# zhangyi-3/UCDIR

Measured on AMD Instinct MI355X. Metric: restored images/sec at 50-step p_sample_loop, 256x256 SID, higher is better.
Workload: dtype bf16

## Files before the change

### ucdir_amd/csrc/engine.hip

```cpp
#include <hip/hip_runtime.h>

#include <algorithm>
#include <cmath>
#include <cstdio>
#include <cstring>
#include <map>
#include <mutex>
#include <set>
#include <array>
#include <atomic>
#include <memory>
#include <string>
#include <vector>

#include "../../include/ucdir_hip.h"
#include "cgemm.hip.h"
#include "conv_halo.hip.h"
#include "akgm_halo.hip.h"
#include "akgm_pre.hip.h"
#include "akgm_ws.hip.h"
#include "akgm_ws32.hip.h"
#include "akgm_ws64.hip.h"
#include "conv_ws.hip.h"
#include "conv_sk.hip.h"
// ... 274 lines not shown
    sd.print([&](int, int n) { fprintf(stderr, "CGEMM TIMING mode=%d TM=%d nk=%d n=%d:", p.cols_mode, TM, p.nk, n); });
}

static int ilog2(int v) { int s = 0; while ((1 << s) < v) ++s; return s; }

static void zero_gemm(GemmP& p) { std::memset(&p, 0, sizeof(p)); p.alpha = 1.f; p.groups_per_wg = 1; }

static Act make_act(DevPool& pool, int B, int H, int W, int C, bool with_stats = true) {
    Act a; a.B = B; a.H = H; a.W = W; a.C = C;
    a.p = (bf16_t*)pool.alloc((size_t)a.elems() * sizeof(bf16_t), true);
    if (with_stats) {
        a.stats = pool.alloc_stats(B);
    }
    return a;
}

static void choose_tile(int H, int W, int& th, int& tw) {
    static std::map<std::pair<int, int>, std::pair<int, int>> memo;
    static std::mutex mu;
    std::lock_guard<std::mutex> lk(mu);
    auto it = memo.find({H, W});
    if (it != memo.end()) { th = it->second.first; tw = it->second.second; return; }
    double best = -1; th = 16; tw = 16;
    for (int a = 1; a <= 64; ++a)
        for (int b = 4; b <= 256; ++b) {
            if (a * b > 256 || (a + 2) * (b + 2) > HC_HALO_PX) continue;
            const double tiles = (double)((H + a - 1) / a) * ((W + b - 1) / b);
            const double util = (double)H * W / (tiles * 256.0) - 1e-4 * (a + 2) * (b + 2) / 324.0;
            if (util > best) { best = util; th = a; tw = b; }
        }
    memo[{H, W}] = {th, tw};
}

static std::atomic<int> g_last_ksplit{0};
template <int TM, bool DUAL = false>
static void launch_halo(GemmP p, hipStream_t st) {
    const int ks = p.ksplit > 1 ? p.ksplit : 1;
    g_last_ksplit = ks;
    const int nblk = p.nbatch * p.tiles_x * p.tiles_y * p.rowtiles * (p.up_phase ? 4 : 1) * ks + p.alt_blocks;
    ProfEntry e = gemm_entry((TM == 128 ? KEY_HALO128 : KEY_HALO64) + (p.up_phase ? KEY_HALO_UP : 0) + (DUAL ? KEY_HALO_DUAL : 0), p, EPI_STD, p.cg);
    if (p.alt_blocks) add_res_rider(e, p);
    StampDump sd(st, STAMPS_256); p.dbg = sd.dbg();
    bracket(e, st, [&] {
        hipLaunchKernelGGL((conv3x3_halo_kernel<TM, DUAL>), dim3(nblk), dim3(HC_THREADS), hc_lds_bytes<TM>(), st, p);
        if (ks == 1) return;
        const long long items = (long long)p.H * p.W * (p.up_phase ? 4 : 1) * (p.nfeat / 8);
        int gx = (int)((items + 255) / 256); if (gx > 1024) gx = 1024;
        hipLaunchKernelGGL(conv_splitk_finish_kernel, dim3(gx, p.nbatch), dim3(256), 0, st, p, TM);
    });
    sd.print([](int, int n) { fprintf(stderr, "TIMING n=%d:", n); });
}

static std::atomic<int> g_persist_grid{0};
static int num_cus() {
    if (g_persist_grid > 0) return g_persist_grid;
    static std::map<int, int> memo;
    static std::mutex mu;
    std::lock_guard<std::mutex> lk(mu);
    int dev = 0;
    HIPC(hipGetDevice(&dev));
    auto it = memo.find(dev);
    if (it != memo.end()) return it->second;
    int n = 0;
    HIPC(hipDeviceGetAttribute(&n, hipDeviceAttributeMultiprocessorCount, dev));
    if (n <= 0) n = 256;
    memo[dev] = n;
    return n;
}

static thread_local float* t_splitk = nullptr;
static float* splitk_scratch() {
    if (t_splitk) return t_splitk;
    std::lock_guard<std::mutex> lk(g_static_mu);
    int dev = 0;
    HIPC(hipGetDevice(&dev));
    auto it = g_splitk_buf.find(dev);
    if (it != g_splitk_buf.end()) return it->second;
    float* sk = nullptr;
    HIPC(hipMalloc((void**)&sk, SCRATCH_BYTES));
    g_splitk_buf[dev] = sk;
    return sk;
}
static std::atomic<int> g_splitk{-1};
static bool splitk_on() {
    return g_splitk < 0 ? env().splitk : g_splitk != 0;
}
static int choose_ksplit(int wgs, int nchunks, int steps_per_chunk, double out_elems) {
    if (!splitk_on() || wgs > env().splitk_wgs || wgs <= 0) return 1;
    const double unsplit = (double)nchunks * steps_per_chunk * (wgs > 256 ? 1.3 : 1.0);
    int best = 1;
    double best_cost = 0.85 * unsplit;
    for (int ks = 2; ks <= 16 && wgs * ks <= SPLITK_MAX_WGS && nchunks / ks >= 2; ++ks) {
        const double steps = (double)((nchunks + ks - 1) / ks) * steps_per_chunk * (wgs * ks > 256 ? 1.3 : 1.0);
        const double cost = steps + 5.0 + out_elems * 4.0 * ks / 1.5e6;
        if (cost < best_cost) { best_cost = cost; best = ks; }
    }
    return best;
}

static int choose_usplit(int nblk) {
    if (!splitk_on() || nblk <= 0) return 1;
    int best_us = 1;
    double best = 1e30;
    for (int us = 1; us <= 4; us *= 2) {
        const double cost = (double)((nblk * us + SPLITK_MAX_WGS - 1) / SPLITK_MAX_WGS) * (1.0 / us + 0.10);
        if (cost < best - 1e-9) { best = cost; best_us = us; }
// ... 827 lines not shown
    for (size_t li = 0; li < c->layers.size(); ++li) {
        const LayerDesc& d = c->layers[li];
        LayerRT& r = c->rt[li];
        for (; si < slots.size() && slots[si].layer == (int)li; ++si) {
            const ActSlot& s = slots[si];
            Act a; a.B = B; a.H = s.H; a.W = s.W; a.C = s.C;
            if (s.id == (int)bufs.size()) bufs.push_back((bf16_t*)c->apool.alloc((size_t)a.elems() * sizeof(bf16_t), true));
            a.p = bufs.at(s.id);
            if (s.which != ACT_RES) a.stats = c->apool.alloc_stats(B);
            (s.which == ACT_OUT ? r.out : s.which == ACT_H1 ? r.h1 : s.which == ACT_RES ? r.res : r.bo) = a;
        }
        if (d.kind == "stem") {
            fl += 2.0 * 9 * d.cin * d.cout * c->Hc * c->Wc;
        } else if (d.kind == "down") {
            const int h = level_dim(c->Hc, d.level + 1), w = level_dim(c->Wc, d.level + 1);
            fl += 2.0 * 9 * d.cin * d.cout * h * w;
        } else if (d.kind == "up") {
            const int h = level_dim(c->Hc, d.level - 1), w = level_dim(c->Wc, d.level - 1);
            fl += 2.0 * 9 * d.cin * d.cout * h * w;
        } else {
            const int h = level_dim(c->Hc, d.level), w = level_dim(c->Wc, d.level);
            r.G = (float*)c->apool.alloc((size_t)B * h * w * 8 * sizeof(float));
            const double hw = (double)h * w;
            fl += 2.0 * 9 * d.cin * d.cout * hw + 2.0 * 9 * d.cout * d.cout * hw;
            if (d.cin != d.cout) fl += 2.0 * d.cin * d.cout * hw;
            fl += 2.0 * hw * (3 * 16 + 72 * 8);
            if (d.attn) {
                if (h * w > maxN) maxN = h * w;
                attC = d.cout;
                fl += 2.0 * d.cout * 3 * d.cout * hw + 2.0 * d.cout * d.cout * hw + 4.0 * hw * hw * d.cout;
            }
        }
    }
    fl += 2.0 * 9 * c->cfg.inner_channel * c->cfg.channel_mults[0] * c->cfg.out_channel * c->Hc * c->Wc;
    c->flops = fl * B;
    c->fin_act = Act();
    if (!c->fin_w || env().no_fused_final) c->fin_act = make_act(c->apool, B, c->Hc, c->Wc, c->cfg.inner_channel * c->cfg.channel_mults[0], false);
    if (maxN > 0) alloc_attn(c->apool, c->attn, B, maxN, attC, c->cfg.attn_fp16 != 0);
    c->attw = (float*)c->apool.alloc((size_t)c->nblocks * B * 8 * sizeof(float));
    {
        int maxC = 0;
        for (const auto& d : c->layers) if (d.kind == "block" && d.cout > maxC) maxC = d.cout;
        c->tcbuf = (float*)c->apool.alloc((size_t)B * (9 * 8 * maxC + 2) * sizeof(float), false);
    }
    c->guide_ready = false;
}

static void forward(ucdir_ctx* c, const float* cond, const float* xt, const float* level, float* eps, hipStream_t st) {
    struct ScratchScope { ScratchScope(float* p) { t_splitk = p; } ~ScratchScope() { t_splitk = nullptr; } } scratch_scope(c->splitk);
    c->apool.zero_stats(st);
    require(c->finalized, "weights not finalized");
    require(c->guide_ready, "ucdir_prepare_guide must be called before ucdir_unet_forward");
    const int B = c->B, inner = c->cfg.inner_channel;
    {
        const size_t sm = (size_t)(6 * inner + c->nblocks * 8) * sizeof(float);
        hipLaunchKernelGGL(time_mlp_kernel, dim3(B), dim3(256), sm, st, level, inner, c->mlp_w1, c->mlp_b1, c->mlp_w2,
                           c->mlp_b2, c->tw, c->nblocks, c->attw, B);
        HIPC(hipGetLastError());
    }
    std::vector<const Act*> skips;
    const Act* cur = nullptr;
    for (size_t li = 0; li < c->layers.size(); ++li) {
        const LayerDesc& d = c->layers[li];
        const LayerW& w = c->lw[li];
        LayerRT& r = c->rt[li];
        if (d.kind == "stem") {
            const int tx = (c->Wc + 15) / 16, ty = (c->Hc + 15) / 16;
            const int units = tx * ty * (d.cout / 64) * B;
            hipLaunchKernelGGL((stem_mfma_kernel<6, 0>), dim3(units < 4 * num_cus() ? units : 4 * num_cus()), dim3(256), 0, st, cond, xt, c->H, c->W,
                               c->Hc, c->Wc, d.cout, tx, w.stem_w, r.out.p, r.out.stats, tx * ty, d.cout / 64, B);
            HIPC(hipGetLastError());
        } else if (d.kind == "down") {
            run_conv(w.conv, COLS_DOWN, {*cur, nullptr, r.out, 0, nullptr, true}, st);
        } else if (d.kind == "up") {
            run_conv(w.conv, COLS_UP, {*cur, nullptr, r.out, 0, nullptr, true}, st);
        } else {
            const Act* x0 = cur; const Act* x1 = nullptr;
            if (d.skip_c) { x1 = skips.back(); skips.pop_back(); require(x1->C == d.skip_c, "skip channel mismatch"); }
            const bool res_done = run_conv(w.conv, COLS_S1, {*x0, x1, r.h1, 1, nullptr, true, w.has_res ? &r.res : nullptr, w.has_res ? &w.resconv : nullptr}, st);
            const Act* res = x0;
            if (w.has_res) { if (!res_done) run_conv(w.resconv, COLS_S1, {*x0, x1, r.res, 0, nullptr, false}, st); res = &r.res; }
            Act& bo = d.attn ? r.bo : r.out;
            run_akgm(w.sp, r.h1, r.G, c->attw + (size_t)w.block_index * B * 8, *res, bo, c->tcbuf, st);
            if (d.attn) run_attention(w.qkv, w.outp, bo, r.out, c->attn, st);
        }
        cur = &r.out;
        if (d.push_skip) skips.push_back(cur);
    }
    {
        const int C = cur->C, co = c->cfg.out_channel;
        if (!env().no_fused_final && c->fin_w) {
            const int tiles = ((c->Wc + 15) / 16) * ((c->Hc + 15) / 16) * B;
            const dim3 grid(tiles < 3 * num_cus() ? tiles : 3 * num_cus());
            const size_t lds = (size_t)324 * 80 + (size_t)9 * (C / 32) * 1024 + (size_t)8 * C + (size_t)8 * B;
            require(lds <= 160 * 1024, "final conv: channel count too large for the fused kernel");
            hipLaunchKernelGGL(final_conv_kernel, grid, dim3(256), lds, st, cur->p, c->Hc, c->Wc, C, cur->stats,
                               1.0 / ((double)C * c->Hc * c->Wc), c->fin_gamma, c->fin_beta, c->fin_w, c->fin_b, co, eps, c->H, c->W, B);
            HIPC(hipGetLastError());
        } else {
            hipLaunchKernelGGL(gn_silu_kernel, dim3(2048, 1, B), dim3(256), 0, st, cur->p, c->fin_act.p, c->Hc, c->Wc, C,
                               cur->stats, 1.0 / ((double)C * c->Hc * c->Wc), c->fin_gamma, c->fin_beta);
            HIPC(hipGetLastError());
            Act dummy; dummy.B = B; dummy.H = c->Hc; dummy.W = c->Wc; dummy.C = c->fin_conv.cout;
            run_conv(c->fin_conv, COLS_S1, {c->fin_act, nullptr, dummy, 0, nullptr, false, nullptr, nullptr, eps, c->H, c->W}, st);
        }
    }
}

static void forward_graph(ucdir_ctx* c, const float* cond, const float* xt, const float* level, float* eps, hipStream_t st) {
    for (auto& f : c->graphs)
        if (f.cond == cond && f.xt == xt && f.lvl == level && f.eps == eps) { c->miss_streak = 0; HIPC(hipGraphLaunch(f.ex, st)); return; }
    const bool same_as_last = c->last_miss[0] == cond && c->last_miss[1] == xt && c->last_miss[2] == level && c->last_miss[3] == eps;
    c->last_miss[0] = cond; c->last_miss[1] = xt; c->last_miss[2] = level; c->last_miss[3] = eps;
    if (c->miss_streak >= 2 && !same_as_last) { ++c->miss_streak; forward(c, cond, xt, level, eps, st); return; }
    ++c->miss_streak;
    if (c->graphs.size() >= 8) { const int ms = c->miss_streak; c->drop_graphs(); c->miss_streak = ms; }
    if (!c->cap_stream) HIPC(hipStreamCreateWithFlags(&c->cap_stream, hipStreamNonBlocking));
    HIPC(hipStreamSynchronize(st));
    ucdir_ctx::FwdGraph f{cond, xt, level, eps, nullptr, nullptr};
    HIPC(hipStreamBeginCapture(c->cap_stream, hipStreamCaptureModeThreadLocal));
    try { forward(c, cond, xt, level, eps, c->cap_stream); }
    catch (...) { hipGraph_t g = nullptr; (void)hipStreamEndCapture(c->cap_stream, &g); if (g) (void)hipGraphDestroy(g); throw; }
    HIPC(hipStreamEndCapture(c->cap_stream, &f.g));
    if (hipGraphInstantiate(&f.ex, f.g, nullptr, nullptr, 0) != hipSuccess) {
        (void)hipGraphDestroy(f.g);
        throw std::runtime_error("hipGraphInstantiate failed for a captured forward");
    }
    c->graphs.push_back(f);
    HIPC(hipGraphLaunch(f.ex, st));
}

extern "C" {

int32_t ucdir_abi_version(void) { return UCDIR_ABI_VERSION; }
const char* ucdir_last_error(void) { return g_err.c_str(); }

int32_t ucdir_create(const ucdir_config* cfg, ucdir_ctx** out) {
    API_BEGIN
    require(cfg && out, "null argument");
    require(cfg->n_mults >= 1 && cfg->n_mults <= UCDIR_MAX_MULTS, "bad n_mults");
    require(cfg->inner_channel % 64 == 0, "inner_channel must be a multiple of 64");
    int ndev = 0;
    hipError_t e = hipGetDeviceCount(&ndev);
    require(e == hipSuccess && ndev > 0, "no HIP device available (libucdir_hip has no CPU fallback)");
    require(cfg->device >= 0 && cfg->device < ndev, "bad device ordinal");
    DevGuard dg(cfg->device);
    ensure_kernel_attrs();
    std::unique_ptr<ucdir_ctx> c(new ucdir_ctx());
    c->cfg = *cfg;
    c->layers = build_layers(*cfg);
    for (const auto& d : c->layers)
// ... 95 lines not shown
int32_t ucdir_set_graph(ucdir_ctx* ctx, int32_t on) {
    API_BEGIN
    require(ctx, "null ctx");
    DevGuard dg(ctx->cfg.device);
    ctx->use_graph = on != 0;
    if (!on) ctx->drop_graphs();
    API_END
}

int32_t ucdir_debug_read(ucdir_ctx* ctx, const char* layer, const char* what, float* dst, int64_t dst_elems, void* stream) {
    API_BEGIN
    require(ctx && layer && what && dst, "null argument");
    DevGuard dg(ctx->cfg.device);
    require(!ctx->acts_reused, "ucdir_debug_read: activation buffers of this (large) shape are recycled by lifetime; set "
                               "UCDIR_KEEP_ACTS=1 before planning to keep every layer's tensor");
    const bool padded = !strncmp(what, "padded:", 7);
    if (padded) what += 7;
    for (size_t li = 0; li < ctx->layers.size(); ++li) {
        if (ctx->layers[li].name != layer) continue;
        const LayerRT& r = ctx->rt[li];
        require(!padded || !strcmp(what, "out") || !strcmp(what, "h1") || !strcmp(what, "res") || !strcmp(what, "bo"),
                "debug_read: padded: takes out, h1, res or bo");
        if (!strcmp(what, "attw")) {
            require(ctx->layers[li].kind == "block" && ctx->attw != nullptr, "attw: not a residual block");
            require(dst_elems == (int64_t)ctx->B * 8, "debug_read: attw has B * 8 elements");
            HIPC(hipMemcpyAsync(dst, ctx->attw + (size_t)ctx->lw[li].block_index * ctx->B * 8, sizeof(float) * ctx->B * 8,
                                hipMemcpyDeviceToDevice, (hipStream_t)stream));
            return 0;
        }
        const Act* a = &r.out;
        if (!strcmp(what, "h1")) a = &r.h1;
        else if (!strcmp(what, "res")) a = &r.res;
        else if (!strcmp(what, "bo")) a = &r.bo;
        require(a->p != nullptr, "no such activation");
        const int64_t n = padded ? (int64_t)a->elems() : (int64_t)a->B * a->C * a->H * a->W;
        require(n == dst_elems, "debug_read: dst has " + std::to_string(dst_elems) + " elements, activation has " + std::to_string(n));
        if (padded) hipLaunchKernelGGL(act_to_nchw_padded_kernel, dim3(2048), dim3(256), 0, (hipStream_t)stream, a->p, dst, a->B, a->C, a->H, a->W);
        else hipLaunchKernelGGL(act_to_nchw_kernel, dim3(2048), dim3(256), 0, (hipStream_t)stream, a->p, dst, a->B, a->C, a->H, a->W);
        HIPC(hipGetLastError());
        return 0;
    }
    throw std::runtime_error(std::string("unknown layer ") + layer);
    API_END
}

int32_t ucdir_debug_flag(const char* name, int32_t value) {
    API_BEGIN
    require(name != nullptr, "null argument");
    if (!strcmp(name, "flash")) g_flash = value;
    else if (!strcmp(name, "splitk")) g_splitk = value;
    else if (!strcmp(name, "skmix")) g_skmix = value;
    else if (!strcmp(name, "convsk")) g_convsk = value;
    else if (!strcmp(name, "persist_grid")) g_persist_grid = value;
    else if (!strcmp(name, "reuse_acts")) g_reuse_acts = value < 0 ? -1 : value != 0;
    else throw std::runtime_error(std::string("unknown debug flag ") + name);
    API_END
}

int32_t ucdir_debug_launch_plan(const char* what, int32_t wgs, int32_t nchunks, int32_t steps_per_chunk, double out_elems) {
    if (!what) return -1;
    try {
        if (!strcmp(what, "ksplit")) return choose_ksplit(wgs, nchunks, steps_per_chunk, out_elems);
        if (!strcmp(what, "usplit")) return choose_usplit(wgs);
        if (!strcmp(what, "last_ksplit")) return g_last_ksplit;
        if (!strcmp(what, "tile")) {
            if (wgs < 1 || nchunks < 1) return -1;
            int th = 0, tw = 0;
            choose_tile(wgs, nchunks, th, tw);
            return th * 1000 + tw;
        }
        if (!strcmp(what, "sk_strips")) {
            if (wgs < 1) return -1;
            int ns = 0, Ws = 0, Wpe = 0, nhp = 0;
            bool ok;
            if (nchunks == 14) ok = conv_sk_strips<1, 4>(wgs, ns, Ws, Wpe, nhp);
            else if (nchunks == 28) ok = conv_sk_strips<2, 8>(wgs, ns, Ws, Wpe, nhp);
            else if (nchunks == 18) ok = conv_sk_strips<1, 8>(wgs, ns, Ws, Wpe, nhp);
            else return -1;
            return ok ? ns * 1000 + nhp : 0;
        }
    } catch (...) {}
    return -1;
}

int32_t ucdir_debug_act_plan(const ucdir_config* cfg, int32_t B, int32_t H, int32_t W, int32_t pad_mode, int32_t reuse, int32_t cap,
                             int32_t* rows) {
    try {
        require(cfg && (rows || cap <= 0), "null argument");
        require(cfg->n_mults >= 1 && cfg->n_mults <= UCDIR_MAX_MULTS, "bad n_mults");
        int Hc, Wc;
        plan_compute_size(*cfg, B, H, W, pad_mode, Hc, Wc);
        const std::vector<ActSlot> plan = act_plan(build_layers(*cfg), Hc, Wc, reuse_acts_mode(reuse < 0 ? -1 : reuse != 0, Hc, Wc));
        for (size_t i = 0; i < plan.size() && (int64_t)i < cap; ++i) {
            const ActSlot& s = plan[i];
            const int32_t r[6] = {s.layer, s.which, s.H, s.W, s.C, s.id};
            for (int k = 0; k < 6; ++k) rows[i * 6 + k] = r[k];
        }
        return (int32_t)plan.size();
    }
    catch (const std::exception& e) { fail(e.what()); }
    catch (...) { fail("unknown error"); }
    return -1;
}

int32_t ucdir_profile_enable(int32_t on) {
    API_BEGIN
// ... 233 lines not shown
    {
        int cinp, coutp;
        auto wp = pad_conv_weight(H_("conv10_1.weight"), 3, {32}, 1, cinp, coutp);
        std::vector<float> w3((size_t)3 * cinp); for (int o = 0; o < 3; ++o) for (int ci = 0; ci < cinp; ++ci) w3[(size_t)o * cinp + ci] = wp[(size_t)o * cinp + ci];
        c->conv["conv10_1"] = upload_conv(c->wpool, w3.data(), H_("conv10_1.bias").data(), nullptr, nullptr, 3, cinp, 1);
    }
    const int ups[4][3] = {{6, 512, 256}, {7, 256, 128}, {8, 128, 64}, {9, 64, 32}};
    for (auto& u : ups) {
        const std::string n = "upv" + std::to_string(u[0]);
        const int cin = u[1], cout = u[2], coutp = pad64(cout);
        const auto& w = H_(n + ".weight"); const auto& b = H_(n + ".bias");
        require(w.size() == (size_t)cin * cout * 4, "predictor: " + n + " size");
        std::vector<float> t((size_t)4 * coutp * cin, 0.f), bb((size_t)4 * coutp, 0.f);
        for (int q = 0; q < 4; ++q) for (int o = 0; o < cout; ++o) {
            bb[(size_t)q * coutp + o] = b[o];
            for (int ci = 0; ci < cin; ++ci) t[((size_t)q * coutp + o) * cin + ci] = w[((size_t)ci * cout + o) * 4 + q];
        }
        c->conv[n] = upload_conv(c->wpool, t.data(), bb.data(), nullptr, nullptr, 4 * coutp, cin, 1);
    }
    c->host.clear();
    c->finalized = true;
}

static void predictor_plan(ucdir_predictor* c, int B, int H, int W) {
    require(B >= 1, "predictor: B must be >= 1");
    require(H >= 33 && W >= 33, "predictor: H, W must be >= 33 (reflect pad)");
    c->apool.release(); c->act.clear();
    c->B = B; c->H = H; c->W = W; c->Hc = (H / 32 + 1) * 32; c->Wc = (W / 32 + 1) * 32;
    const int ch[5] = {64, 64, 128, 256, 512};
    for (int l = 0; l < 5; ++l) {
        const int h = c->Hc >> l, w = c->Wc >> l;
        const std::string L = std::to_string(l + 1);
        c->act["a" + L] = make_act(c->apool, B, h, w, ch[l], false);
        c->act["c" + L] = make_act(c->apool, B, h, w, ch[l], false);
        if (l < 4) c->act["p" + L] = make_act(c->apool, B, h / 2, w / 2, ch[l], false);
    }
    for (int l = 3; l >= 0; --l) {
        const int h = c->Hc >> l, w = c->Wc >> l;
        const std::string L = std::to_string(9 - l);
        c->act["u" + L] = make_act(c->apool, B, h, w, ch[l], false);
        c->act["a" + L] = make_act(c->apool, B, h, w, ch[l], false);
        c->act["c" + L] = make_act(c->apool, B, h, w, ch[l], false);
    }
}

static void predictor_forward(ucdir_predictor* c, const float* x, float* y, hipStream_t st) {
    const int B = c->B;
    auto A = [&](const std::string& n) -> Act& { return c->act.at(n); };
    auto CV = [&](const std::string& n) -> const ConvW& { return c->conv.at(n); };
    {
        const int tx = (c->Wc + 15) / 16, ty = (c->Hc + 15) / 16;
        const int units = tx * ty * B;
        hipLaunchKernelGGL((stem_mfma_kernel<3, 2>), dim3(units < 4 * num_cus() ? units : 4 * num_cus()), dim3(256), 0, st, x, x, c->H, c->W, c->Hc, c->Wc, 64, tx,
                           c->in_w, A("a1").p, (stat_t*)nullptr, tx * ty, 1, B);
        HIPC(hipGetLastError());
    }
    run_conv(CV("conv1_2"), COLS_S1, {A("a1"), nullptr, A("c1"), 2, nullptr, false}, st);
    for (int l = 1; l <= 4; ++l) {
        const std::string L = std::to_string(l), N = std::to_string(l + 1);
        Act& src = A("c" + L); Act& dst = A("p" + L);
        hipLaunchKernelGGL(maxpool2_kernel, dim3(2048), dim3(256), 0, st, src.p, dst.p, B, src.H, src.W, src.C);
        HIPC(hipGetLastError());
        run_conv(CV("conv" + N + "_1"), COLS_S1, {dst, nullptr, A("a" + N), 2, nullptr, false}, st);
        run_conv(CV("conv" + N + "_2"), COLS_S1, {A("a" + N), nullptr, A("c" + N), 2, nullptr, false}, st);
    }
    const Act* cur = &A("c5");
    for (int l = 6; l <= 9; ++l) {
        const std::string L = std::to_string(l);
        Act& up = A("u" + L);
        const ConvW& w = CV("upv" + L);
        {
            GemmP p; zero_gemm(p);
            p.A = w.A; p.a_ld = w.Kpad; p.a_rows = w.rows_pad;
            p.B0 = cur->p; p.b0_bstride = cur->bstride(); p.ld0 = cur->C; p.c0 = cur->C;
            p.cols_mode = COLS_S1; p.H = cur->H; p.W = cur->W; p.Wp = cur->W + 2; p.Hi = cur->H; p.Wi = cur->W; p.Wpi = p.Wp;
            p.p0 = p.Wp + 1; p.pn = (cur->H - 1) * p.Wp + cur->W;
            p.ntaps = 1; p.cg = cur->C; p.cpt = cur->C / 8; p.nk = w.Kpad / CG_BK;
            p.tiles = (p.pn + CG_TP - 1) / CG_TP; p.rowtiles = w.rows_pad / w.TM; p.nbatch = B;
            p.bias = w.bias; p.nfeat = w.cout; p.shuffle_c = up.C;
            p.out = up.p; p.out_bstride = up.bstride(); p.out_ld = up.C;
            launch_cgemm(p, w.TM, EPI_STD, st);
        }
        const Act& skip = A("c" + std::to_string(10 - l));
        run_conv(CV("conv" + L + "_1"), COLS_S1, {up, &skip, A("a" + L), 2, nullptr, false}, st);
        run_conv(CV("conv" + L + "_2"), COLS_S1, {A("a" + L), nullptr, A("c" + L), 2, nullptr, false}, st);
        cur = &A("c" + L);
    }
    {
        const ConvW& w = CV("conv10_1");
        GemmP p; zero_gemm(p);
        p.A = w.A; p.a_ld = w.Kpad; p.a_rows = w.rows_pad;
        p.B0 = cur->p; p.b0_bstride = cur->bstride(); p.ld0 = cur->C; p.c0 = cur->C;
        p.cols_mode = COLS_S1; p.H = cur->H; p.W = cur->W; p.Wp = cur->W + 2; p.Hi = cur->H; p.Wi = cur->W; p.Wpi = p.Wp;
        p.p0 = p.Wp + 1; p.pn = (cur->H - 1) * p.Wp + cur->W;
        p.ntaps = 1; p.cg = cur->C; p.cpt = cur->C / 8; p.nk = w.Kpad / CG_BK;
        p.tiles = (p.pn + CG_TP - 1) / CG_TP; p.rowtiles = w.rows_pad / w.TM; p.nbatch = B;
        p.bias = w.bias; p.nfeat = 3; p.out = y; p.out_nchw = 1; p.crop_h = c->H; p.crop_w = c->W;
        launch_cgemm(p, w.TM, EPI_STD, st);
    }
}

extern "C" {

int32_t ucdir_predictor_create(int32_t device, ucdir_predictor** out) {
    API_BEGIN
    require(out, "null argument");
    int ndev = 0;
// ... 80 lines not shown
```

### ucdir_amd/csrc/misc.hip.h

```cpp
#pragma once
#include "common.h"

__global__ void act_stats_kernel(const bf16_t* __restrict__ x, int H, int W, int C, stat_t* __restrict__ stats) {
    const int b = blockIdx.x;
    const int Wp = W + 2;
    const long long bs = (long long)(H + 2) * Wp * C;
    const int c8 = C / 8;
    double s1 = 0, s2 = 0;
    for (long long i = threadIdx.x; i < (long long)H * W * c8; i += blockDim.x) {
        int c = (int)(i % c8);
        long long pix = i / c8;
        int y = (int)(pix / W), xx = (int)(pix % W);
        const uint4 v = *reinterpret_cast<const uint4*>(x + b * bs + ((long long)(y + 1) * Wp + xx + 1) * C + c * 8);
        const bf16_t* h = reinterpret_cast<const bf16_t*>(&v);
#pragma unroll
        for (int k = 0; k < 8; ++k) { float f = bf2f(h[k]); s1 += f; s2 += (double)f * f; }
    }
    __shared__ double sh[2][256];
    sh[0][threadIdx.x] = s1; sh[1][threadIdx.x] = s2;
    __syncthreads();
    for (int o = 128; o > 0; o >>= 1) {
        if ((int)threadIdx.x < o) { sh[0][threadIdx.x] += sh[0][threadIdx.x + o]; sh[1][threadIdx.x] += sh[1][threadIdx.x + o]; }
        __syncthreads();
    }
    if (threadIdx.x == 0) stat_store(stats, b, sh[0][0], sh[1][0]);
}

__global__ void nchw_to_act_kernel(const float* __restrict__ src, bf16_t* __restrict__ dst, int B, int C, int H, int W) {
    long long n = (long long)B * H * W * C;
    for (long long i = blockIdx.x * (long long)blockDim.x + threadIdx.x; i < n; i += (long long)gridDim.x * blockDim.x) {
        int c = (int)(i % C); long long t = i / C;
        int x = (int)(t % W); t /= W;
        int y = (int)(t % H); int b = (int)(t / H);
        float v = src[(((long long)b * C + c) * H + y) * W + x];
        dst[(((long long)b * (H + 2) + y + 1) * (W + 2) + x + 1) * C + c] = f2bf(v);
    }
}
__global__ void act_to_nchw_kernel(const bf16_t* __restrict__ src, float* __restrict__ dst, int B, int C, int H, int W) {
    long long n = (long long)B * H * W * C;
    for (long long i = blockIdx.x * (long long)blockDim.x + threadIdx.x; i < n; i += (long long)gridDim.x * blockDim.x) {
        int x = (int)(i % W); long long t = i / W;
        int y = (int)(t % H); t /= H;
        int c = (int)(t % C); int b = (int)(t / C);
        dst[i] = bf2f(src[(((long long)b * (H + 2) + y + 1) * (W + 2) + x + 1) * C + c]);
    }
}
__global__ void act_to_nchw_padded_kernel(const bf16_t* __restrict__ src, float* __restrict__ dst, int B, int C, int H, int W) {
    const int Hp = H + 2, Wp = W + 2;
    long long n = (long long)B * Hp * Wp * C;
    for (long long i = blockIdx.x * (long long)blockDim.x + threadIdx.x; i < n; i += (long long)gridDim.x * blockDim.x) {
        int x = (int)(i % Wp); long long t = i / Wp;
        int y = (int)(t % Hp); t /= Hp;
        int c = (int)(t % C); int b = (int)(t / C);
        dst[i] = bf2f(src[(((long long)b * Hp + y) * Wp + x) * C + c]);
    }
}
__global__ void nchw8_to_compact_kernel(const float* __restrict__ src, float* __restrict__ dst, int B, int H, int W) {
    long long n = (long long)B * H * W * 8;
    for (long long i = blockIdx.x * (long long)blockDim.x + threadIdx.x; i < n; i += (long long)gridDim.x * blockDim.x) {
        int s = (int)(i % 8); long long t = i / 8;
        long long pix = t % ((long long)H * W); int b = (int)(t / ((long long)H * W));
        dst[i] = src[((long long)b * 8 + s) * H * W + pix];
    }
}

__device__ __forceinline__ int reflect_idx(int i, int n) { return i < n ? i : 2 * (n - 1) - i; }

template <int CIN, int ACT>
__global__ __launch_bounds__(256, 4) void stem_mfma_kernel(const float* __restrict__ cond, const float* __restrict__ xt,
                                                           int H, int W, int Hc, int Wc, int C0, int tiles_x,
                                                           const bf16_t* __restrict__ wfrag,
                                                           bf16_t* __restrict__ out, stat_t* __restrict__ stats_out,
                                                           int tiles, int ncb, int nb) {
    __shared__ uint4 halo[324];
    __shared__ uint4 wl[2 * 5 * 64];
    __shared__ float red[8];
    __shared__ __attribute__((aligned(16))) unsigned char otile[4 * 32 * 144];
    const int tid = threadIdx.x, lane = tid & 63, wv = tid >> 6, hh = lane >> 5;
    const int total = tiles * ncb * nb;
    auto gather = [&](int u, float (&v)[2][8]) {
        const int tile = u % tiles, b = u / (tiles * ncb);
        const int y0 = (tile / tiles_x) * 16, x0 = (tile % tiles_x) * 16;
#pragma unroll
        for (int uu = 0; uu < 2; ++uu) {
            const int hp = tid + uu * 256;
#pragma unroll
            for (int k = 0; k < 8; ++k) v[uu][k] = 0.f;
            if (hp < 324) {
                const int hr = hp / 18, hc = hp - hr * 18;
                const int yy = y0 + hr - 1, xx = x0 + hc - 1;
                if (yy >= 0 && yy < Hc && xx >= 0 && xx < Wc) {
                    const int ys = reflect_idx(yy, H), xs = reflect_idx(xx, W);
#pragma unroll
                    for (int ci = 0; ci < CIN; ++ci) {
                        const float* src = ci < 3 ? cond : xt;
                        v[uu][ci] = src[(((long long)b * 3 + (ci % 3)) * H + ys) * W + xs];
                    }
                }
            }
        }
    };
    float v[2][8];
    if ((int)blockIdx.x < total) gather(blockIdx.x, v);
    int cb_cur = -1;
#pragma unroll 1
    for (int u = blockIdx.x; u < total; u += gridDim.x) {
        const int tile = u % tiles, cb = (u / tiles) % ncb, b = u / (tiles * ncb);
        const int y0 = (tile / tiles_x) * 16, x0 = (tile % tiles_x) * 16;
        __syncthreads();
#pragma unroll
        for (int uu = 0; uu < 2; ++uu)
            if (tid + uu * 256 < 324) halo[tid + uu * 256] = pack8_bf16(v[uu]);
        if (cb != cb_cur) {
            for (int i = tid; i < 2 * 5 * 64; i += 256)
                wl[i] = *reinterpret_cast<const uint4*>(wfrag + ((long long)cb * 2 * 5 * 64 + i) * 8);
            cb_cur = cb;
        }
        if (u + (int)gridDim.x < total) gather(u + gridDim.x, v);
        __syncthreads();
        int hp0[2];
#pragma unroll
        for (int tp = 0; tp < 2; ++tp) {
            const int slot = tp * 32 + (lane & 31);
            hp0[tp] = (wv * 4 + (slot >> 4)) * 18 + (slot & 15);
        }
        f32x16_t acc[2][2];
#pragma unroll
        for (int tm = 0; tm < 2; ++tm)
#pragma unroll
            for (int tp = 0; tp < 2; ++tp)
#pragma unroll
                for (int e = 0; e < 16; ++e) acc[tm][tp][e] = 0.f;
#pragma unroll 1
        for (int j = 0; j < 5; ++j) {
            const int t0 = 2 * j, t1 = (2 * j + 1 > 8) ? 8 : 2 * j + 1;
            const int sh = hh ? (t1 / 3) * 18 + (t1 % 3) : (t0 / 3) * 18 + (t0 % 3);
            bf16x8_t af[2], bfr[2];
#pragma unroll
            for (int tm = 0; tm < 2; ++tm) af[tm] = *reinterpret_cast<const bf16x8_t*>(&wl[(tm * 5 + j) * 64 + lane]);
#pragma unroll
            for (int tp = 0; tp < 2; ++tp) {
                bfr[tp] = *reinterpret_cast<const bf16x8_t*>(&halo[hp0[tp] + sh]);
                if (j == 4 && hh) bfr[tp] = __builtin_bit_cast(bf16x8_t, make_uint4(0x3F803F80u, 0u, 0u, 0u));
            }
#pragma unroll
            for (int tm = 0; tm < 2; ++tm)
#pragma unroll
                for (int tp = 0; tp < 2; ++tp)
                    acc[tm][tp] = __builtin_amdgcn_mfma_f32_32x32x16_bf16(af[tm], bfr[tp], acc[tm][tp], 0, 0, 0);
        }
        float s1 = 0.f, s2 = 0.f;
        unsigned char* ot = otile + wv * (32 * 144);
#pragma unroll
        for (int tp = 0; tp < 2; ++tp) {
            {
                const int slot = lane & 31;
                const int y = y0 + wv * 4 + tp * 2 + (slot >> 4), x = x0 + (slot & 15);
                const bool inb = y < Hc && x < Wc;
#pragma unroll
                for (int tm = 0; tm < 2; ++tm)
#pragma unroll
                    for (int g = 0; g < 4; ++g) {
                        const int ch = tm * 32 + 8 * g + 4 * hh;
                        float vv[4] = {acc[tm][tp][4 * g + 0], acc[tm][tp][4 * g + 1], acc[tm][tp][4 * g + 2], acc[tm][tp][4 * g + 3]};
#pragma unroll
                        for (int i = 0; i < 4; ++i) {
                            if (ACT == 2) vv[i] = fmaxf(0.2f * vv[i], vv[i]);
                            if (inb) { s1 += vv[i]; s2 += vv[i] * vv[i]; }
                        }
                        *reinterpret_cast<uint2*>(ot + slot * 144 + ch * 2) = make_uint2(pack2_bf16(vv[0], vv[1]), pack2_bf16(vv[2], vv[3]));
                    }
// ... 5 lines not shown
                if (y < Hc && x < Wc)
                    *reinterpret_cast<uint4*>(out + (((long long)b * (Hc + 2) + y + 1) * (Wc + 2) + x + 1) * C0 + cb * 64 + c16 * 8) =
                        *reinterpret_cast<const uint4*>(ot + slot * 144 + c16 * 16);
            }
        }
        if (stats_out) {
            for (int off = 32; off > 0; off >>= 1) { s1 += __shfl_xor(s1, off); s2 += __shfl_xor(s2, off); }
            if (lane == 0) { red[wv * 2] = s1; red[wv * 2 + 1] = s2; }
            __syncthreads();
            if (tid == 0) stat_add(stats_out, b, red[0] + red[2] + red[4] + red[6], red[1] + red[3] + red[5] + red[7]);
        }
    }
}

__global__ __launch_bounds__(256) void gn_silu_kernel(const bf16_t* __restrict__ x, bf16_t* __restrict__ y, int H, int W, int C,
                                                      const stat_t* __restrict__ stats, double inv_count,
                                                      const float* __restrict__ gamma, const float* __restrict__ beta) {
    const int b = blockIdx.z;
    float mean, rstd;
    {
        double S, Q;
        stat_read(stats, nullptr, b, S, Q);
        double m = S * inv_count;
        double var = Q * inv_count - m * m;
        if (var < 0) var = 0;
        mean = (float)m; rstd = (float)(1.0 / sqrt(var + 1e-5));
    }
    const int c8n = C / 8;
    const long long bs = (long long)(H + 2) * (W + 2) * C;
    const long long n = (long long)H * W * c8n;
    for (long long i = blockIdx.x * (long long)blockDim.x + threadIdx.x; i < n; i += (long long)gridDim.x * blockDim.x) {
        const int c = (int)(i % c8n) * 8;
        const long long pix = i / c8n;
        const int yy = (int)(pix / W), xx = (int)(pix % W);
        const long long off = b * bs + ((long long)(yy + 1) * (W + 2) + xx + 1) * C + c;
        const uint4 v = *reinterpret_cast<const uint4*>(x + off);
        const bf16_t* h = reinterpret_cast<const bf16_t*>(&v);
        const float4 g0 = *reinterpret_cast<const float4*>(gamma + c), g1 = *reinterpret_cast<const float4*>(gamma + c + 4);
        const float4 b0 = *reinterpret_cast<const float4*>(beta + c), b1 = *reinterpret_cast<const float4*>(beta + c + 4);
        const float gg[8] = {g0.x, g0.y, g0.z, g0.w, g1.x, g1.y, g1.z, g1.w};
        const float bb[8] = {b0.x, b0.y, b0.z, b0.w, b1.x, b1.y, b1.z, b1.w};
        float fv[8];
#pragma unroll
        for (int k = 0; k < 8; ++k) fv[k] = silu_fast((bf2f(h[k]) - mean) * rstd * gg[k] + bb[k]);
        *reinterpret_cast<uint4*>(y + off) = pack8_bf16(fv);
    }
}

typedef __attribute__((ext_vector_type(4))) float f32x4_t;
__global__ __launch_bounds__(256) void final_conv_kernel(const bf16_t* __restrict__ x, int H, int W, int C,
                                                         const stat_t* __restrict__ stats, double inv_count,
                                                         const float* __restrict__ gamma, const float* __restrict__ beta,
                                                         const bf16_t* __restrict__ wfrag, const float* __restrict__ bias, int cout,
                                                         float* __restrict__ out, int crop_h, int crop_w, int nb) {
    extern __shared__ __attribute__((aligned(16))) unsigned char fsm[];
    constexpr int RS = 80;
    unsigned char* wl = fsm + 324 * RS;
    const int nc32 = C / 32, nstep = 9 * nc32;
    for (int it = threadIdx.x; it < nstep * 64; it += 256)
        *reinterpret_cast<uint4*>(wl + it * 16) = *reinterpret_cast<const uint4*>(wfrag + (long long)it * 8);
    float* gb = reinterpret_cast<float*>(wl + nstep * 1024);
    float* ms = gb + 2 * C;
    for (int i = threadIdx.x; i < nb; i += 256) {
        double S, Q;
        float mean, rstd;
        stat_read(stats, nullptr, i, S, Q);
        mean_rstd(S, Q, inv_count, mean, rstd);
        ms[2 * i] = mean; ms[2 * i + 1] = rstd;
    }
    __syncthreads();
    const int lane = threadIdx.x & 63, wv = threadIdx.x >> 6;
    const int col = lane & 15, kg = lane >> 4;
    const int tiles_x = (W + 15) >> 4, tiles_y = (H + 15) >> 4, tps = tiles_x * tiles_y, total = nb * tps;
    int b_cur = -1;
    for (int t = blockIdx.x; t < total; t += gridDim.x) {
        const int b = t / tps, r = t - b * tps, ty = r / tiles_x, tx = r - ty * tiles_x;
        const int x0 = tx * 16, y0 = ty * 16;
        const bf16_t* xb = x + (long long)b * (H + 2) * (W + 2) * C;
        uint4 v[6]; int dst[6]; long long src[6];
#pragma unroll
        for (int u = 0; u < 6; ++u) {
            const int it = threadIdx.x + u * 256;
            dst[u] = -1; src[u] = 0;
            if (it < 324 * 4) {
                const int hp = it >> 2, c = (it & 3) * 8;
                const int hr = hp / 18, hc = hp - hr * 18;
                const int gy = y0 + hr - 1, gx = x0 + hc - 1;
                dst[u] = (hp * RS + c * 2) | ((gy >= 0 && gy < H && gx >= 0 && gx < W) ? 0 : (1 << 30));
                src[u] = ((long long)(gy + 1) * (W + 2) + gx + 1) * C + c;
            }
        }
        auto request = [&](int c32) {
#pragma unroll
            for (int u = 0; u < 6; ++u) {
                v[u] = make_uint4(0, 0, 0, 0);
                if (dst[u] >= 0 && !(dst[u] >> 30)) v[u] = *reinterpret_cast<const uint4*>(xb + src[u] + c32 * 32);
            }
        };
        request(0);
        if (b != b_cur) {
            const float mean = ms[2 * b], rstd = ms[2 * b + 1];
            for (int i = threadIdx.x; i < C; i += 256) { const float sc = rstd * gamma[i]; gb[i] = sc; gb[C + i] = beta[i] - mean * sc; }
            b_cur = b;
        }
        f32x4_t acc[4];
#pragma unroll
        for (int tq = 0; tq < 4; ++tq) acc[tq] = (f32x4_t){0.f, 0.f, 0.f, 0.f};
        for (int c32 = 0; c32 < nc32; ++c32) {
            __syncthreads();
#pragma unroll
            for (int u = 0; u < 6; ++u) {
                if (dst[u] < 0) continue;
                uint4 o = make_uint4(0, 0, 0, 0);
                const int off = dst[u] & ((1 << 30) - 1);
                if (!(dst[u] >> 30)) {
                    const int c = c32 * 32 + ((threadIdx.x + u * 256) & 3) * 8;
                    const bf16_t* h = reinterpret_cast<const bf16_t*>(&v[u]);
                    float fv[8];
#pragma unroll
                    for (int k = 0; k < 8; ++k) fv[k] = silu_fast(fmaf(bf2f(h[k]), gb[c + k], gb[C + c + k]));
                    o = pack8_bf16(fv);
                }
                *reinterpret_cast<uint4*>(fsm + off) = o;
            }
            if (c32 + 1 < nc32) request(c32 + 1);
            __syncthreads();
            for (int tap = 0; tap < 9; ++tap) {
                const int ky = tap / 3, kx = tap - 3 * ky;
                const bf16x8_t af = *reinterpret_cast<const bf16x8_t*>(wl + ((tap * nc32 + c32) * 64 + lane) * 16);
#pragma unroll
                for (int tq = 0; tq < 4; ++tq) {
                    const int hp = (wv * 4 + tq + ky) * 18 + col + kx;
                    const bf16x8_t bf = *reinterpret_cast<const bf16x8_t*>(fsm + hp * RS + kg * 16);
                    acc[tq] = __builtin_amdgcn_mfma_f32_16x16x32_bf16(af, bf, acc[tq], 0, 0, 0);
                }
            }
        }
        if (kg == 0) {
            const int xx = x0 + col;
#pragma unroll
            for (int tq = 0; tq < 4; ++tq) {
                const int y = y0 + wv * 4 + tq;
                if (y < crop_h && xx < crop_w) {
#pragma unroll
                    for (int o = 0; o < 4; ++o)
                        if (o < cout) out[(((long long)b * cout + o) * crop_h + y) * crop_w + xx] = acc[tq][o] + bias[o];
                }
            }
        }
    }
}

__global__ __launch_bounds__(256) void time_mlp_kernel(const float* __restrict__ level, int inner,
                                                       const float* __restrict__ w1, const float* __restrict__ b1,
                                                       const float* __restrict__ w2, const float* __restrict__ b2,
                                                       const float* __restrict__ tw, int nblocks,
                                                       float* __restrict__ attw , int B) {
    extern __shared__ float tsm[];
    float* enc = tsm;
    float* h1 = tsm + inner;
    float* temb = h1 + 4 * inner;
    float* hid = temb + inner;
    const int b = blockIdx.x;
    const float lv = level[b];
    const int half = inner / 2;
    for (int k = threadIdx.x; k < half; k += 256) {
        const float step = (float)k / (float)half;
        const float e = lv * expf(-9.210340371976184f * step);
        enc[k] = sinf(e); enc[k + half] = cosf(e);
    }
    __syncthreads();
    for (int o = threadIdx.x; o < 4 * inner; o += 256) {
        float a = b1[o];
        for (int k = 0; k < inner; ++k) a += w1[o * inner + k] * enc[k];
        h1[o] = a / (1.0f + expf(-a));
    }
    __syncthreads();
    for (int o = threadIdx.x; o < inner; o += 256) {
        float a = b2[o];
        for (int k = 0; k < 4 * inner; ++k) a += w2[o * 4 * inner + k] * h1[k];
        temb[o] = a;
    }
    __syncthreads();
    const int per = 8 * inner + 8 + 64 + 8;
    for (int i = threadIdx.x; i < nblocks * 8; i += 256) {
        const int l = i / 8, o = i % 8;
        const float* W0 = tw + (long long)l * per;
        float a = W0[8 * inner + o];
        for (int k = 0; k < inner; ++k) a += W0[o * inner + k] * temb[k];
        hid[i] = a / (1.0f + expf(-a));
    }
    __syncthreads();
    for (int i = threadIdx.x; i < nblocks * 8; i += 256) {
        const int l = i / 8, o = i % 8;
        const float* W2 = tw + (long long)l * per + 8 * inner + 8;
        float a = W2[64 + o];
        for (int k = 0; k < 8; ++k) a += W2[o * 8 + k] * hid[l * 8 + k];
        attw[((long long)l * B + b) * 8 + o] = a;
    }
}

__global__ __launch_bounds__(256) void guide_branch_kernel(const float* __restrict__ guide, int H, int W, int Hc, int Wc,
                                                           int k, const float* __restrict__ gw, float* __restrict__ G) {
// ... 187 lines not shown
```

Baseline: 36.90.

## Fold time MLP into stem kernel blocks and skip cropped final-conv tiles

The time-embedding MLP now runs inside extra leading blocks of the stem kernel instead of as its own launch. It reuses the stem's shared memory and stages the w2 rows through LDS. The final fused conv now covers only tiles that overlap the cropped output region (H,W) rather than the padded (Hc,Wc) extent, which skips work whose results are discarded. Optional timing stamps are also added under a compile-time flag. The costs are a more complex stem kernel with heterogeneous blocks, and the MLP rows are computed by only B blocks.

Result: no change. 37.01, median of 6 (+0.3%).

```diff
diff --git a/ucdir_amd/csrc/engine.hip b/ucdir_amd/csrc/engine.hip
--- a/ucdir_amd/csrc/engine.hip
+++ b/ucdir_amd/csrc/engine.hip
@@ -350,6 +350,8 @@
 }
 
 static std::atomic<int> g_persist_grid{0};
+static std::atomic<int> g_final_all_tiles{-1};
+static std::atomic<int> g_head_mlp{-1};
 static int num_cus() {
     if (g_persist_grid > 0) return g_persist_grid;
     static std::map<int, int> memo;
@@ -1283,7 +1285,8 @@
     require(c->finalized, "weights not finalized");
     require(c->guide_ready, "ucdir_prepare_guide must be called before ucdir_unet_forward");
     const int B = c->B, inner = c->cfg.inner_channel;
-    {
+    const bool mlp_in_stem = g_head_mlp != 0 && !c->layers.empty() && c->layers[0].kind == "stem" && time_mlp_fits_stem(inner, c->nblocks);
+    if (!mlp_in_stem) {
         const size_t sm = (size_t)(6 * inner + c->nblocks * 8) * sizeof(float);
         hipLaunchKernelGGL(time_mlp_kernel, dim3(B), dim3(256), sm, st, level, inner, c->mlp_w1, c->mlp_b1, c->mlp_w2,
                            c->mlp_b2, c->tw, c->nblocks, c->attw, B);
@@ -1298,8 +1301,11 @@
         if (d.kind == "stem") {
             const int tx = (c->Wc + 15) / 16, ty = (c->Hc + 15) / 16;
             const int units = tx * ty * (d.cout / 64) * B;
-            hipLaunchKernelGGL((stem_mfma_kernel<6, 0>), dim3(units < 4 * num_cus() ? units : 4 * num_cus()), dim3(256), 0, st, cond, xt, c->H, c->W,
-                               c->Hc, c->Wc, d.cout, tx, w.stem_w, r.out.p, r.out.stats, tx * ty, d.cout / 64, B);
+            const bool mlp = mlp_in_stem && li == 0;
+            const TimeMlpArgs ma{level, c->mlp_w1, c->mlp_b1, c->mlp_w2, c->mlp_b2, c->tw, c->attw, inner, c->nblocks, mlp ? B : 0};
+            int cap = 4 * num_cus() - ma.nb; if (cap < 1) cap = 1;
+            hipLaunchKernelGGL((stem_mfma_kernel<6, 0>), dim3((units < cap ? units : cap) + ma.nb), dim3(256), 0, st, cond, xt, c->H, c->W,
+                               c->Hc, c->Wc, d.cout, tx, w.stem_w, r.out.p, r.out.stats, tx * ty, d.cout / 64, B, ma);
             HIPC(hipGetLastError());
         } else if (d.kind == "down") {
             run_conv(w.conv, COLS_DOWN, {*cur, nullptr, r.out, 0, nullptr, true}, st);
@@ -1321,13 +1327,18 @@
     {
         const int C = cur->C, co = c->cfg.out_channel;
         if (!env().no_fused_final && c->fin_w) {
-            const int tiles = ((c->Wc + 15) / 16) * ((c->Hc + 15) / 16) * B;
+            const bool all = g_final_all_tiles == 1;
+            const int live_x = ((all ? c->Wc : c->W) + 15) / 16, live_y = ((all ? c->Hc : c->H) + 15) / 16;
+            const int tiles = live_x * live_y * B;
             const dim3 grid(tiles < 3 * num_cus() ? tiles : 3 * num_cus());
             const size_t lds = (size_t)324 * 80 + (size_t)9 * (C / 32) * 1024 + (size_t)8 * C + (size_t)8 * B;
             require(lds <= 160 * 1024, "final conv: channel count too large for the fused kernel");
+            StampDump sd(st, STAMPS_256);
             hipLaunchKernelGGL(final_conv_kernel, grid, dim3(256), lds, st, cur->p, c->Hc, c->Wc, C, cur->stats,
-                               1.0 / ((double)C * c->Hc * c->Wc), c->fin_gamma, c->fin_beta, c->fin_w, c->fin_b, co, eps, c->H, c->W, B);
+                               1.0 / ((double)C * c->Hc * c->Wc), c->fin_gamma, c->fin_beta, c->fin_w, c->fin_b, co, eps, c->H, c->W, B,
+                               live_x, live_y, sd.dbg());
             HIPC(hipGetLastError());
+            sd.print([&](int, int n) { fprintf(stderr, "TIMING final_conv C=%d tiles=%d grid=%d n=%d (per tile: C/32 x [stage+activate, mfma], then store + next tile's setup):", C, tiles, (int)grid.x, n); });
         } else {
             hipLaunchKernelGGL(gn_silu_kernel, dim3(2048, 1, B), dim3(256), 0, st, cur->p, c->fin_act.p, c->Hc, c->Wc, C,
                                cur->stats, 1.0 / ((double)C * c->Hc * c->Wc), c->fin_gamma, c->fin_beta);
@@ -1529,6 +1540,8 @@
     else if (!strcmp(name, "skmix")) g_skmix = value;
     else if (!strcmp(name, "convsk")) g_convsk = value;
     else if (!strcmp(name, "persist_grid")) g_persist_grid = value;
+    else if (!strcmp(name, "final_all_tiles")) g_final_all_tiles = value;
+    else if (!strcmp(name, "head_mlp")) g_head_mlp = value;
     else if (!strcmp(name, "reuse_acts")) g_reuse_acts = value < 0 ? -1 : value != 0;
     else throw std::runtime_error(std::string("unknown debug flag ") + name);
     API_END
@@ -1868,7 +1881,7 @@
         const int tx = (c->Wc + 15) / 16, ty = (c->Hc + 15) / 16;
         const int units = tx * ty * B;
         hipLaunchKernelGGL((stem_mfma_kernel<3, 2>), dim3(units < 4 * num_cus() ? units : 4 * num_cus()), dim3(256), 0, st, x, x, c->H, c->W, c->Hc, c->Wc, 64, tx,
-                           c->in_w, A("a1").p, (stat_t*)nullptr, tx * ty, 1, B);
+                           c->in_w, A("a1").p, (stat_t*)nullptr, tx * ty, 1, B, TimeMlpArgs{});
         HIPC(hipGetLastError());
     }
     run_conv(CV("conv1_2"), COLS_S1, {A("a1"), nullptr, A("c1"), 2, nullptr, false}, st);
diff --git a/ucdir_amd/csrc/misc.hip.h b/ucdir_amd/csrc/misc.hip.h
--- a/ucdir_amd/csrc/misc.hip.h
+++ b/ucdir_amd/csrc/misc.hip.h
@@ -66,17 +66,121 @@
 
 __device__ __forceinline__ int reflect_idx(int i, int n) { return i < n ? i : 2 * (n - 1) - i; }
 
+struct TimeMlpArgs {
+    const float* level; const float* w1; const float* b1; const float* w2; const float* b2; const float* tw;
+    float* attw;
+    int inner, nblocks, nb;
+};
+constexpr int TIME_MLP_VEC_FLOATS = 2 * 5 * 64 * 4;
+constexpr int TIME_MLP_STAGE_FLOATS = 4 * 32 * 144 / 4;
+static inline bool time_mlp_fits_stem(int inner, int nblocks) {
+    return inner % 32 == 0 && 6 * inner + 8 * nblocks <= TIME_MLP_VEC_FLOATS;
+}
+
+__device__ __forceinline__ float dot_row_direct(const float* __restrict__ w, const float* x, int K, float a) {
+    for (int k0 = 0; k0 < K; k0 += 32) {
+        float4 v[8];
+#pragma unroll
+        for (int j = 0; j < 8; ++j) v[j] = *reinterpret_cast<const float4*>(w + k0 + 4 * j);
+#pragma unroll
+        for (int j = 0; j < 8; ++j) {
+            a += v[j].x * x[k0 + 4 * j]; a += v[j].y * x[k0 + 4 * j + 1];
+            a += v[j].z * x[k0 + 4 * j + 2]; a += v[j].w * x[k0 + 4 * j + 3];
+        }
+    }
+    return a;
+}
+
+template <typename Row, typename Init, typename Store>
+__device__ __forceinline__ void staged_rows_dot(int R, int K, Row row, const float* x, float* stage, Init init, Store store) {
+    const int tid = threadIdx.x;
+    for (int r0 = 0; r0 < R; r0 += 256) {
+        const int rg = R - r0 < 256 ? R - r0 : 256;
+        int kc = 1 << (31 - __clz(TIME_MLP_STAGE_FLOATS / rg - 1));
+        if (kc > K) kc = K;
+        const int ld = kc + 1;
+        float a = tid < rg ? init(r0 + tid) : 0.f;
+        for (int k0 = 0; k0 < K; k0 += kc) {
+            const int kn = K - k0 < kc ? K - k0 : kc, q = kn >> 2, n4 = rg * q;
+            __syncthreads();
+            for (int i0 = 0; i0 < n4; i0 += 4 * 256) {
+                float4 v[4];
+#pragma unroll
+                for (int j = 0; j < 4; ++j) {
+                    const int i = i0 + j * 256 + tid, rr = i / q;
+                    if (i < n4) v[j] = *reinterpret_cast<const float4*>(row(r0 + rr) + k0 + 4 * (i - rr * q));
+                }
+#pragma unroll
+                for (int j = 0; j < 4; ++j) {
+                    const int i = i0 + j * 256 + tid, rr = i / q;
+                    float* d = stage + rr * ld + 4 * (i - rr * q);
+                    if (i < n4) { d[0] = v[j].x; d[1] = v[j].y; d[2] = v[j].z; d[3] = v[j].w; }
+                }
+            }
+            __syncthreads();
+            if (tid < rg) {
+#pragma unroll 16
+                for (int kk = 0; kk < kn; ++kk) a += stage[tid * ld + kk] * x[k0 + kk];
+            }
+        }
+        if (tid < rg) store(r0 + tid, a);
+    }
+    __syncthreads();
+}
+
+__device__ __forceinline__ void time_mlp_staged(const TimeMlpArgs& m, int b, float* vec, float* stage) {
+    const int inner = m.inner, nblocks = m.nblocks;
+    float* enc = vec;
+    float* h1 = vec + inner;
+    float* temb = h1 + 4 * inner;
+    float* hid = temb + inner;
+    const float lv = m.level[b];
+    const int half = inner / 2;
+    for (int k = threadIdx.x; k < half; k += 256) {
+        const float step = (float)k / (float)half;
+        const float e = lv * expf(-9.210340371976184f * step);
+        enc[k] = sinf(e); enc[k + half] = cosf(e);
+    }
+    __syncthreads();
+    for (int o = threadIdx.x; o < 4 * inner; o += 256) {
+        const float a = dot_row_direct(m.w1 + (long long)o * inner, enc, inner, m.b1[o]);
+        h1[o] = a / (1.0f + expf(-a));
+    }
+    staged_rows_dot(inner, 4 * inner, [&](int o) { return m.w2 + (long long)o * 4 * inner; }, h1, stage,
+                    [&](int o) { return m.b2[o]; }, [&](int o, float a) { temb[o] = a; });
+    const int per = 8 * inner + 8 + 64 + 8;
+    for (int i = threadIdx.x; i < nblocks * 8; i += 256) {
+        const float* W0 = m.tw + (long long)(i / 8) * per;
+        const float a = dot_row_direct(W0 + (i % 8) * inner, temb, inner, W0[8 * inner + (i % 8)]);
+        hid[i] = a / (1.0f + expf(-a));
+    }
+    __syncthreads();
+    for (int i = threadIdx.x; i < nblocks * 8; i += 256) {
+        const int l = i / 8, o = i % 8;
+        const float* W2 = m.tw + (long long)l * per + 8 * inner + 8;
+        float a = W2[64 + o];
+        for (int k = 0; k < 8; ++k) a += W2[o * 8 + k] * hid[l * 8 + k];
+        m.attw[((long long)l * m.nb + b) * 8 + o] = a;
+    }
+}
+
 template <int CIN, int ACT>
 __global__ __launch_bounds__(256, 4) void stem_mfma_kernel(const float* __restrict__ cond, const float* __restrict__ xt,
                                                            int H, int W, int Hc, int Wc, int C0, int tiles_x,
                                                            const bf16_t* __restrict__ wfrag,
                                                            bf16_t* __restrict__ out, stat_t* __restrict__ stats_out,
-                                                           int tiles, int ncb, int nb) {
+                                                           int tiles, int ncb, int nb, TimeMlpArgs mlp) {
     __shared__ uint4 halo[324];
     __shared__ uint4 wl[2 * 5 * 64];
     __shared__ float red[8];
     __shared__ __attribute__((aligned(16))) unsigned char otile[4 * 32 * 144];
+    if ((int)blockIdx.x < mlp.nb) {
+        __builtin_amdgcn_s_setprio(3);
+        time_mlp_staged(mlp, blockIdx.x, reinterpret_cast<float*>(wl), reinterpret_cast<float*>(otile));
+        return;
+    }
     const int tid = threadIdx.x, lane = tid & 63, wv = tid >> 6, hh = lane >> 5;
+    const int g0 = (int)blockIdx.x - mlp.nb, gn = (int)gridDim.x - mlp.nb;
     const int total = tiles * ncb * nb;
     auto gather = [&](int u, float (&v)[2][8]) {
         const int tile = u % tiles, b = u / (tiles * ncb);
@@ -101,10 +205,10 @@
         }
     };
     float v[2][8];
-    if ((int)blockIdx.x < total) gather(blockIdx.x, v);
+    if (g0 < total) gather(g0, v);
     int cb_cur = -1;
 #pragma unroll 1
-    for (int u = blockIdx.x; u < total; u += gridDim.x) {
+    for (int u = g0; u < total; u += gn) {
         const int tile = u % tiles, cb = (u / tiles) % ncb, b = u / (tiles * ncb);
         const int y0 = (tile / tiles_x) * 16, x0 = (tile % tiles_x) * 16;
         __syncthreads();
@@ -116,7 +220,7 @@
                 wl[i] = *reinterpret_cast<const uint4*>(wfrag + ((long long)cb * 2 * 5 * 64 + i) * 8);
             cb_cur = cb;
         }
-        if (u + (int)gridDim.x < total) gather(u + gridDim.x, v);
+        if (u + gn < total) gather(u + gn, v);
         __syncthreads();
         int hp0[2];
 #pragma unroll
@@ -228,7 +332,15 @@
                                                          const stat_t* __restrict__ stats, double inv_count,
                                                          const float* __restrict__ gamma, const float* __restrict__ beta,
                                                          const bf16_t* __restrict__ wfrag, const float* __restrict__ bias, int cout,
-                                                         float* __restrict__ out, int crop_h, int crop_w, int nb) {
+                                                         float* __restrict__ out, int crop_h, int crop_w, int nb,
+                                                         int live_x, int live_y, unsigned long long* dbg) {
+#ifdef UCDIR_TIMING
+    const bool dbg_on = dbg && blockIdx.x == gridDim.x / 2 && threadIdx.x == 0;
+    int dbg_n = 0;
+#define FC_STAMP() do { if (dbg_on && dbg_n < 250) dbg[dbg_n++] = __builtin_amdgcn_s_memtime(); } while (0)
+#else
+#define FC_STAMP() do {} while (0)
+#endif
     extern __shared__ __attribute__((aligned(16))) unsigned char fsm[];
     constexpr int RS = 80;
     unsigned char* wl = fsm + 324 * RS;
@@ -247,10 +359,10 @@
     __syncthreads();
     const int lane = threadIdx.x & 63, wv = threadIdx.x >> 6;
     const int col = lane & 15, kg = lane >> 4;
-    const int tiles_x = (W + 15) >> 4, tiles_y = (H + 15) >> 4, tps = tiles_x * tiles_y, total = nb * tps;
+    const int tps = live_x * live_y, total = nb * tps;
     int b_cur = -1;
     for (int t = blockIdx.x; t < total; t += gridDim.x) {
-        const int b = t / tps, r = t - b * tps, ty = r / tiles_x, tx = r - ty * tiles_x;
+        const int b = t / tps, r = t - b * tps, ty = r / live_x, tx = r - ty * live_x;
         const int x0 = tx * 16, y0 = ty * 16;
         const bf16_t* xb = x + (long long)b * (H + 2) * (W + 2) * C;
         uint4 v[6]; int dst[6]; long long src[6];
@@ -284,6 +396,7 @@
         for (int tq = 0; tq < 4; ++tq) acc[tq] = (f32x4_t){0.f, 0.f, 0.f, 0.f};
         for (int c32 = 0; c32 < nc32; ++c32) {
             __syncthreads();
+            FC_STAMP();
 #pragma unroll
             for (int u = 0; u < 6; ++u) {
                 if (dst[u] < 0) continue;
@@ -301,6 +414,7 @@
             }
             if (c32 + 1 < nc32) request(c32 + 1);
             __syncthreads();
+            FC_STAMP();
             for (int tap = 0; tap < 9; ++tap) {
                 const int ky = tap / 3, kx = tap - 3 * ky;
                 const bf16x8_t af = *reinterpret_cast<const bf16x8_t*>(wl + ((tap * nc32 + c32) * 64 + lane) * 16);
@@ -312,6 +426,7 @@
                 }
             }
         }
+        FC_STAMP();
         if (kg == 0) {
             const int xx = x0 + col;
 #pragma unroll
@@ -325,6 +440,10 @@
             }
         }
     }
+#ifdef UCDIR_TIMING
+    if (dbg_on) dbg[255] = dbg_n;
+#endif
+#undef FC_STAMP
 }
 
 __global__ __launch_bounds__(256) void time_mlp_kernel(const float* __restrict__ level, int inner,
```
